# HyeonwooNoh/RAU_VQA

Hardware: AMD Instinct MI355X
Metric: QA-pairs/sec fwd+bwd, Ours_SS 8-step RAU, batch 256, 14x14x512 (higher is better)
Workload: dtype f32; 1 GPU; Ours_SS 8-step RAU fwd+bwd, 14x14x512, configs[1]; batch_per_gpu=256, global_batch=256, T=26, feature_map=14x14x512, hops=8, parallelism=dp1, collective=none, hop_weights=SS (x nHop), arithmetic=f32 operands, f32 MFMA accumulate, dropout=train mode, Philox masks per step and rank, launch=eager, 3 streams

## Files before the change

### rau_vqa_amd/csrc/gemm_lin.hip

```cpp
#include <algorithm>
#include <cstdio>
#include <cstdlib>

#include "gemm_core.h"
#include "kernels.h"

namespace rau {

constexpr int BK = 32;
constexpr int BKS = 16;

static GemmParams lin_params(int M, int N, int K, const float* A, long lda, const float* W,
                             long ldw, float* C, long ldc, const LinOpts& o) {
  GemmParams P{};
  P.M = M; P.N = N; P.K = K;
  P.nk = (K + BK - 1) / BK;
  P.A = A; P.a_rs = lda;
  P.B = W; P.b_rs = ldw;
  P.C = C; P.c_rs = ldc;
  P.bias = o.bias; P.bias2 = o.bias2;
  P.addend = o.addend; P.add_rs = o.add_rs;
  P.accumulate = o.accumulate; P.act = o.act;
  P.ymul = o.ymul; P.y_rs = o.y_rs;
  P.emask = o.emask; P.emask_e0 = o.emask_e0; P.emscale = o.emscale;
  P.alpha = o.alpha;
  P.round16 = lin_bf16();
  return P;
}

static int skinny_splits(int M, int N, int K, const LinOpts& o) {
  if (!o.slab) return 1;
  const int tiles = ((M + 63) / 64) * ((N + 63) / 64);
  const int nk = (K + BKS - 1) / BKS;
  constexpr int target = 160;
  int s = (target + tiles - 1) / tiles;
  if (s > nk / 2) s = nk / 2;
  if (s < 1) s = 1;
  while (s > 1 && (size_t)s * M * N > o.slab_floats) --s;
  const int per = (nk + s - 1) / s;
  return (nk + per - 1) / per;
}

template <int ASRC, int BSRC>
static hipError_t lin_gemm(hipStream_t st, int M, int N, int K, const float* A, long lda,
                           const float* W, long ldw, float* C, long ldc, const LinOpts& o) {
  GemmParams P = lin_params(M, N, K, A, lda, W, ldw, C, ldc, o);
  if ((long)M * N >= 128L * 128 * 256 && !o.defer_splits)
    return launch_gemm<128, 128, BK, ASRC, BSRC, EPI_LIN>(st, P, 1);
  if (o.slab && skinny_dma_ok(M, K, lda, ldw, BSRC == SRC_RC, 1, &N, &A, &W)) {
    const int tiles = ((M + 63) / 64) * ((N + 63) / 64);
    const int s = skinny_dma_splits(M, K, tiles, (size_t)N, o.slab_floats);
    if ((size_t)s * M * N <= o.slab_floats && (s > 1 || o.defer_splits)) {
      const long off = 0;
      hipError_t e = skinny_dma(st, BSRC == SRC_RC, 1, M, K, &A, lda, &W, ldw, &N, o.slab, &off, s);
      if (e != hipSuccess) return e;
      if (o.defer_splits) {
        *o.defer_splits = s;
        return hipSuccess;
      }
      return lin_reduce_epilogue(st, M, N, s, o.slab, C, ldc, o);
    }
  }
#ifdef RAU_DEV_HOOKS
  if (std::getenv("RAU_LIN_TRACE"))
    std::fprintf(stderr, "lin_gemm fallback %s M=%d N=%d K=%d lda=%ld ldw=%ld slab=%d\n",
                 BSRC == SRC_RC ? "nn" : "nt", M, N, K, lda, ldw, o.slab != nullptr);
#endif
  P.nk = (K + BKS - 1) / BKS;
  const int s = skinny_splits(M, N, K, o);
  if (o.defer_splits) {
    if (!o.slab || (size_t)s * M * N > o.slab_floats) return hipErrorInvalidValue;
    P.C = o.slab;
    P.c_rs = N;
    P.slab_stride = (long)M * N;
    *o.defer_splits = s;
    return launch_gemm<64, 64, BKS, ASRC, BSRC, EPI_SLAB>(st, P, s);
  }
  if (s <= 1) return launch_gemm<64, 64, BKS, ASRC, BSRC, EPI_LIN>(st, P, 1);
  P.C = o.slab;
  P.c_rs = N;
  P.slab_stride = (long)M * N;
  hipError_t e = launch_gemm<64, 64, BKS, ASRC, BSRC, EPI_SLAB>(st, P, s);
  if (e != hipSuccess) return e;
  return lin_reduce_epilogue(st, M, N, s, o.slab, C, ldc, o);
}

hipError_t gemm_nt(hipStream_t st, int M, int N, int K, const float* A, long lda,
                   const float* W, long ldw, float* C, long ldc, const LinOpts& o) {
  return lin_gemm<SRC_KC, SRC_KC>(st, M, N, K, A, lda, W, ldw, C, ldc, o);
}

hipError_t gemm_nn(hipStream_t st, int M, int N, int K, const float* A, long lda,
                   const float* W, long ldw, float* C, long ldc, const LinOpts& o) {
  return lin_gemm<SRC_KC, SRC_RC>(st, M, N, K, A, lda, W, ldw, C, ldc, o);
}

template <int ASRC, int BSRC>
static hipError_t batched_deferred(hipStream_t st, int nb, int M, int N, int K,
                                   const float* const* A, long lda, const float* const* W,
                                   long ldw, float* slab, size_t slab_floats, int* splits) {
  if (nb < 1 || nb > 3) return hipErrorInvalidValue;
  {
    const int Ns[3] = {N, N, N};
    if (skinny_dma_ok(M, K, lda, ldw, BSRC == SRC_RC, nb, Ns, A, W)) {
      const int tiles = ((M + 63) / 64) * ((N + 63) / 64);
      const int s = skinny_dma_splits(M, K, nb * tiles, (size_t)nb * N, slab_floats);
      if ((size_t)nb * s * M * N <= slab_floats) {
        long off[3];
        for (int i = 0; i < nb; ++i) off[i] = (long)i * s * M * N;
        *splits = s;
        return skinny_dma(st, BSRC == SRC_RC, nb, M, K, A, lda, W, ldw, Ns, slab, off, s);
      }
    }
  }
#ifdef RAU_DEV_HOOKS
  if (std::getenv("RAU_LIN_TRACE"))
    std::fprintf(stderr, "batched fallback %s nb=%d M=%d N=%d K=%d slab_floats=%zu\n", BSRC == SRC_RC ? "nn" : "nt",
                 nb, M, N, K, slab_floats);
#endif
  LinOpts o;
  o.slab = slab;
  o.slab_floats = slab_floats / nb;
  GemmParams P = lin_params(M, N, K, A[0], lda, W[0], ldw, slab, N, o);
  P.nk = (K + BKS - 1) / BKS;
  const int s = skinny_splits(M, N, K, o);
  if ((size_t)nb * s * M * N > slab_floats) return hipErrorInvalidValue;
  P.nbatch = nb;
  for (int i = 0; i < nb; ++i) { P.Ab[i] = A[i]; P.Bb[i] = W[i]; }
  P.C = slab;
  P.c_rs = N;
  P.slab_stride = (long)M * N;
  P.slab_batch_stride = (long)s * M * N;
  *splits = s;
  return launch_gemm<64, 64, BKS, ASRC, BSRC, EPI_SLAB>(st, P, s);
}
hipError_t gemm_nt_batched_deferred(hipStream_t st, int nb, int M, int N, int K,
                                    const float* const* A, long lda, const float* const* W,
                                    long ldw, float* slab, size_t slab_floats, int* splits) {
  return batched_deferred<SRC_KC, SRC_KC>(st, nb, M, N, K, A, lda, W, ldw, slab, slab_floats, splits);
}
hipError_t gemm_nn_batched_deferred(hipStream_t st, int nb, int M, int N, int K,
                                    const float* const* A, long lda, const float* const* W,
                                    long ldw, float* slab, size_t slab_floats, int* splits) {
  return batched_deferred<SRC_KC, SRC_RC>(st, nb, M, N, K, A, lda, W, ldw, slab, slab_floats, splits);
}

hipError_t gemm_nt_hetero_deferred(hipStream_t st, int nb, int M, int K, const float* A, long lda,
                                   const float* const* W, long ldw, const int* N, float* slab,
                                   size_t slab_floats, int* splits, size_t* off) {
  if (nb < 1 || nb > 3) return hipErrorInvalidValue;
  int nmax = 0, tiles = 0;
  size_t nsum = 0;
  for (int i = 0; i < nb; ++i) {
    nmax = N[i] > nmax ? N[i] : nmax;
    tiles += ((M + 63) / 64) * ((N[i] + 63) / 64);
    nsum += (size_t)N[i];
  }
  {
    const float* As[3] = {A, A, A};
    if (skinny_dma_ok(M, K, lda, ldw, false, nb, N, As, W)) {
      const int s = skinny_dma_splits(M, K, tiles, nsum, slab_floats);
      if ((size_t)s * M * nsum <= slab_floats) {
        long o2[3];
        size_t acc = 0;
        for (int i = 0; i < nb; ++i) {
          o2[i] = (long)acc;
          off[i] = acc;
          acc += (size_t)s * M * N[i];
        }
        *splits = s;
        return skinny_dma(st, false, nb, M, K, As, lda, W, ldw, N, slab, o2, s);
      }
    }
  }
#ifdef RAU_DEV_HOOKS
  if (std::getenv("RAU_LIN_TRACE"))
    std::fprintf(stderr, "hetero fallback nb=%d M=%d K=%d N=%d,%d,%d\n", nb, M, K, N[0], nb > 1 ? N[1] : 0, nb > 2 ? N[2] : 0);
#endif
  const int nk = (K + BKS - 1) / BKS;
  int s = (160 * nb + tiles - 1) / tiles;
  if (s > nk / 2) s = nk / 2;
  if (s < 1) s = 1;
  while (s > 1 && (size_t)s * M * nsum > slab_floats) --s;
  if ((size_t)s * M * nsum > slab_floats) return hipErrorInvalidValue;
  {
    const int per = (nk + s - 1) / s;
    s = (nk + per - 1) / per;
  }
  LinOpts o;
  GemmParams P = lin_params(M, nmax, K, A, lda, W[0], ldw, slab, nmax, o);
  P.nk = nk;
  P.nbatch = nb;
  size_t acc = 0;
  for (int i = 0; i < nb; ++i) {
    P.Ab[i] = A;
    P.Bb[i] = W[i];
    P.Nb[i] = N[i];
    P.slab_off[i] = (long)acc;
    off[i] = acc;
    acc += (size_t)s * M * N[i];
  }
  *splits = s;
  return launch_gemm<64, 64, BKS, SRC_KC, SRC_KC, EPI_SLAB>(st, P, s);
}

static int tn_splits(int M, int N, int K) {
  const int tiles = ((M + 127) / 128) * ((N + 127) / 128);
  const int nk = (K + BK - 1) / BK;
  constexpr int target = 512;
  int s = target / tiles;
  if (s > nk / 8) s = nk / 8;
  if (s < 1) s = 1;
  const int per = (nk + s - 1) / s;
  return (nk + per - 1) / per;
}
size_t gemm_tn_slab_floats(int M, int N, int K) {
  const int s = tn_splits(M, N, K);
  return (s > 1 ? (size_t)s * M * N : 0) + (size_t)s * M;
}
hipError_t gemm_tn_acc(hipStream_t st, int M, int N, int K, const float* A, long lda,
                       const float* B, long ldb, float* C, long ldc, float* slab, float* dbias, int bf16) {
  LinOpts o;
  o.accumulate = 1;
  const int s = tn_splits(M, N, K);
  float* rs = dbias ? slab + (s > 1 ? (size_t)s * M * N : 0) : nullptr;
  hipError_t e;
  if (s <= 1) {
    GemmParams P = lin_params(M, N, K, A, lda, B, ldb, C, ldc, o);
    P.rs_out = rs;
    if (bf16)
      e = dbias ? launch_gemm<128, 128, BK, SRC_RC_SUM, SRC_RC, EPI_LIN, 1>(st, P, 1)
                : launch_gemm<128, 128, BK, SRC_RC, SRC_RC, EPI_LIN, 1>(st, P, 1);
    else
    e = dbias ? launch_gemm<128, 128, BK, SRC_RC_SUM, SRC_RC, EPI_LIN>(st, P, 1)
              : launch_gemm<128, 128, BK, SRC_RC, SRC_RC, EPI_LIN>(st, P, 1);
  } else {
    if (ldc != N) return hipErrorInvalidValue;
    GemmParams P = lin_params(M, N, K, A, lda, B, ldb, slab, N, o);
    P.slab_stride = (long)M * N;
    P.rs_out = rs;
    if (bf16)
      e = dbias ? launch_gemm<128, 128, BK, SRC_RC_SUM, SRC_RC, EPI_SLAB, 1>(st, P, s)
                : launch_gemm<128, 128, BK, SRC_RC, SRC_RC, EPI_SLAB, 1>(st, P, s);
    else
    e = dbias ? launch_gemm<128, 128, BK, SRC_RC_SUM, SRC_RC, EPI_SLAB>(st, P, s)
              : launch_gemm<128, 128, BK, SRC_RC, SRC_RC, EPI_SLAB>(st, P, s);
    if (e != hipSuccess) return e;
    e = splitk_reduce_acc(st, (size_t)M * N, s, slab, (size_t)M * N, C);
  }
  if (e != hipSuccess || !dbias) return e;
  return splitk_reduce_acc(st, (size_t)M, s, rs, (size_t)M, dbias);
}

static int group_splits(const TnProblem* pr, int np, int K) {
  int tiles = 0;
  for (int i = 0; i < np; ++i) tiles += ((pr[i].M + 127) / 128) * ((pr[i].N + 127) / 128);
  const int nk = (K + BK - 1) / BK;
  constexpr int target = 0;
  const int smax = std::max(1, nk / 16);
  int s = 1;
  if (target > 0) {
    s = (target + tiles / 2) / (tiles > 0 ? tiles : 1);
    s = std::min(std::max(s, 1), smax);
  } else {
    double best = -1.0;
    for (int c = 1; c <= smax; ++c) {
      const int wgs = tiles * c;
      const double eff = (double)wgs / (512.0 * ((wgs + 511) / 512));
      if (eff > best + 0.02) { best = eff; s = c; }
    }
  }
  const int per = (nk + s - 1) / s;
  return (nk + per - 1) / per;
}
size_t gemm_tn_group_slab_floats(const TnProblem* pr, int np, int K) {
  const int s = group_splits(pr, np, K);
  size_t n = 0;
  for (int i = 0; i < np; ++i) n += (size_t)s * ((size_t)pr[i].M * pr[i].N + pr[i].M);
  return n;
}

struct GroupReduce {
  int np, splits;
  long e0[kGroupMax + 1];
  long b0[kGroupMax + 1];
  const float* slab[kGroupMax]; const float* rs[kGroupMax];
  float* dst[kGroupMax]; float* db[kGroupMax];
  long mn[kGroupMax]; int m[kGroupMax];
};
__global__ void k_group_reduce_acc(const GroupReduce R) {
  const long nW = R.e0[R.np], nB = R.b0[R.np];
  for (long i = blockIdx.x * (long)blockDim.x + threadIdx.x; i < nW + nB;
       i += (long)gridDim.x * blockDim.x) {
    const bool bias = i >= nW;
    const long j = bias ? i - nW : i;
    const long* pre = bias ? R.b0 : R.e0;
    int p = 0;
    while (p + 1 < R.np && j >= pre[p + 1]) ++p;
    const long k = j - pre[p];
    if (bias) {
      if (!R.db[p]) continue;
      float v = R.db[p][k];
      for (int s = 0; s < R.splits; ++s) v += R.rs[p][(long)s * R.m[p] + k];
      R.db[p][k] = v;
    } else {
      float v = R.dst[p][k];
      for (int s = 0; s < R.splits; ++s) v += R.slab[p][(long)s * R.mn[p] + k];
      R.dst[p][k] = v;
    }
  }
}

hipError_t gemm_tn_group_acc(hipStream_t st, const TnProblem* pr, int np, int K, float* slab,
                             size_t slab_floats, int bf16) {
  if (np < 1 || np > kGroupMax) return hipErrorInvalidValue;
  if (gemm_tn_group_slab_floats(pr, np, K) > slab_floats) return hipErrorInvalidValue;
  const int s = group_splits(pr, np, K);
  GroupParams G{};
  GroupReduce R{};
  G.np = np; G.K = K;
  G.nk = (K + BK - 1) / BK;
  G.nk_per_split = (G.nk + s - 1) / s;
  R.np = np; R.splits = s;
  float* w = slab;
  int wg = 0;
  for (int i = 0; i < np; ++i) {
    GroupProb& q = G.p[i];
    q.A = pr[i].A; q.lda = pr[i].lda; q.B = pr[i].B; q.ldb = pr[i].ldb;
    q.M = pr[i].M; q.N = pr[i].N;
    q.tiles_m = (q.M + 127) / 128; q.tiles_n = (q.N + 127) / 128;
    q.slab = w;
    w += (size_t)s * q.M * q.N;
    q.rs_out = w;
    w += (size_t)s * q.M;
    G.wg0[i] = wg;
    wg += q.tiles_m * q.tiles_n * s;
    R.slab[i] = q.slab; R.rs[i] = q.rs_out; R.dst[i] = pr[i].C; R.db[i] = pr[i].dbias;
    R.mn[i] = (long)q.M * q.N; R.m[i] = q.M;
    R.e0[i + 1] = R.e0[i] + R.mn[i];
    R.b0[i + 1] = R.b0[i] + q.M;
  }
  G.wg0[np] = wg;
  if (bf16)
    hipLaunchKernelGGL((gemm_group_kernel<128, 128, BK, SRC_RC_SUM, SRC_RC, 1>), dim3(wg), dim3(256), 0,
                       st, G);
  else
  hipLaunchKernelGGL((gemm_group_kernel<128, 128, BK, SRC_RC_SUM, SRC_RC>), dim3(wg), dim3(256), 0,
                     st, G);
  hipError_t e = hipGetLastError();
  if (e != hipSuccess) return e;
  const long n = R.e0[np] + R.b0[np];
  const int blocks = (int)std::min<long>((n + 255) / 256, 2048);
  hipLaunchKernelGGL(k_group_reduce_acc, dim3(blocks), dim3(256), 0, st, R);
  return hipGetLastError();
}

}
```

### rau_vqa_amd/csrc/kernels.h

```cpp
#pragma once
#include <hip/hip_runtime.h>
#include <stddef.h>
#include <stdint.h>

#include "../../include/rau.h"

namespace rau {

constexpr long kMaxSplits = 4096;
constexpr hipError_t kSplitStateError = hipErrorIllegalState;
void split_ws_register(const float* base, size_t floats);
void split_ws_unregister(const float* base);
bool split_span_ok(const float* slab, long nsplit, size_t per_split_floats);

struct LinOpts {
  const float* bias = nullptr;
  const float* bias2 = nullptr;
  const float* addend = nullptr;
  long add_rs = 0;
  int accumulate = 0;
  int act = 0;
  const float* ymul = nullptr;
  long y_rs = 0;
  const uint32_t* emask = nullptr;
  size_t emask_e0 = 0;
  float emscale = 1.f;
  float alpha = 1.f;
  float* slab = nullptr;
  size_t slab_floats = 0;
  int* defer_splits = nullptr;
};
hipError_t gemm_nt(hipStream_t st, int M, int N, int K, const float* A, long lda,
                   const float* W, long ldw, float* C, long ldc, const LinOpts& o);
hipError_t gemm_nn(hipStream_t st, int M, int N, int K, const float* A, long lda,
                   const float* W, long ldw, float* C, long ldc, const LinOpts& o);
hipError_t gemm_nt_batched_deferred(hipStream_t st, int nb, int M, int N, int K,
                                    const float* const* A, long lda, const float* const* W,
                                    long ldw, float* slab, size_t slab_floats, int* splits);
hipError_t gemm_nn_batched_deferred(hipStream_t st, int nb, int M, int N, int K,
                                    const float* const* A, long lda, const float* const* W,
                                    long ldw, float* slab, size_t slab_floats, int* splits);
hipError_t gemm_nt_hetero_deferred(hipStream_t st, int nb, int M, int K, const float* A, long lda,
                                   const float* const* W, long ldw, const int* N, float* slab,
                                   size_t slab_floats, int* splits, size_t* off);
size_t gemm_tn_slab_floats(int M, int N, int K);
hipError_t gemm_tn_acc(hipStream_t st, int M, int N, int K, const float* A, long lda,
                       const float* B, long ldb, float* C, long ldc, float* slab,
                       float* dbias = nullptr, int bf16 = 0);

struct TnProblem {
  int M, N; const float* A; long lda; const float* B; long ldb; float* C; float* dbias;
};
size_t gemm_tn_group_slab_floats(const TnProblem* pr, int np, int K);
hipError_t gemm_tn_group_acc(hipStream_t st, const TnProblem* pr, int np, int K, float* slab,
                             size_t slab_floats, int bf16 = 0);

hipError_t conv_embed_fwd(hipStream_t st, int nB, int D, int S, int M, const float* X,
                          const float* WiT , const float* bi, float* I, int bf16 = 0,
                          int one_per_cu = 0 );
hipError_t conv_embed_fwd_b16(hipStream_t st, int nB, int D, int S, int M, const void* X16,
                              const void* WiT16, const float* bi, float* I);
hipError_t conv_att_pre_b16(hipStream_t st, int nB, int M, int S, int A, const float* I,
                            const void* WpT16, const float* bp, float* Pout);
hipError_t conv_att_pre(hipStream_t st, int nB, int M, int S, int A, const float* I,
                        const float* WpT , const float* bp, float* P, int bf16 = 0,
                        int one_per_cu = 0);
bool conv_sample_ok(int S, int which);
hipError_t conv_sample(hipStream_t st, int epi, int nB, int M, int K, int S, const float* Wt,
                       long w_rs, const float* X, long x_bs, float* C, long c_bs,
                       const float* bias, int act, const float* dj, const float* av,
                       const float* Y = nullptr, float* rs = nullptr, int c16 = 0);
bool conv_wide_ok(int M, int K, int S, long w_rs);
hipError_t conv_wide(hipStream_t st, int epi, int nB, int M, int K, int S, const float* Wt, long w_rs,
                     const float* X, long x_bs, float* C, long c_bs, const float* bias, int act,
                     const float* dj, const float* av, const float* Y, float* rs, int c16, int per_cu);
hipError_t transpose2d(hipStream_t st, int rows, int cols, const float* in, float* out,
                       void* out16 = nullptr);
hipError_t conv_att_dgrad(hipStream_t st, int nB, int M, int S, int A, const float* dS,
                          const float* Wp, const float* dj, const float* a, float* dI,
                          int bf16 = 0);
bool conv_dz_fused_ok(int S, int M, int bf16);
hipError_t conv_att_dgrad_dz(hipStream_t st, int nB, int M, int S, int A, const float* dS,
                             const float* Wp, const float* dj, const float* a, const float* I,
                             float* dZ, float* rs, int dz16 = 0,
                             int bf16 = 0,
                             int ds16 = 0,
                             int light = 0);
bool dgrad16_ok(int M, int K, int S, long w_rs);
hipError_t dgrad16(hipStream_t st, int nB, int M, int K, int S, const float* Wt, long w_rs,
                   const void* X, long x_bs, void* C, long c_bs, const float* dj, const float* av,
                   const float* Y, float* rs, int c16, int x16 = 0 );
bool dgrad_dma_ok(int M, int K, int S, long w_rs);
hipError_t dgrad_dma(hipStream_t st, int nB, int M, int K, int S, const float* Wt, long w_rs,
                     const float* X, long x_bs, float* C, long c_bs, const float* dj, const float* av,
                     const float* Y, float* rs);
hipError_t conv_att_wgrad_ds16(hipStream_t st, int nB, int M, int S, int A, const void* dS16,
                               const float* I, float* dWp, float* slab);
hipError_t conv_embed_dgrad(hipStream_t st, int nB, int D, int S, int M, const float* dZ,
                            const float* Wi, float* dX);
size_t conv_wgrad_slab_floats(int nB, int rowsA, int rowsB, int S);
bool wgrad16_ok(int ra, int rb, int S);
size_t wgrad16_slab_floats(int nB, int ra, int rb, int S);
hipError_t wgrad16(hipStream_t st, int nB, int ra, int rb, int S, const void* A16, long a_bs,
                   const void* B16, long b_bs, float* dW, float* slab);
bool skinny_dma_ok(int M, int K, long lda, long ldb, bool brc, int nprob, const int* N,
                   const float* const* A, const float* const* B);
int skinny_dma_splits(int M, int K, int tiles_all, size_t cols_all, size_t slab_floats);
void skinny_dma_set_deep(int on);
void lin_set_bf16(int on);
int lin_bf16();
hipError_t skinny_dma(hipStream_t st, bool brc, int nprob, int M, int K, const float* const* A,
                      long lda, const float* const* B, long ldb, const int* N, float* slab,
                      const long* off, int splits);
bool wgrad_dma_ok(int ra, int rb, int S);
hipError_t wgrad_dma(hipStream_t st, int nB, int ra, int rb, int S, const float* A, long a_bs,
                     const float* B, long b_bs, float* dW, float* slab, int splits);
hipError_t conv_att_wgrad(hipStream_t st, int nB, int M, int S, int A, const float* dS,
                          const float* I, float* dWp, float* slab, int bf16 = 0);
hipError_t conv_embed_wgrad(hipStream_t st, int nB, int D, int S, int M, const float* dI,
                            const float* I, const float* X, float* dWi, float* slab,
                            int bf16 = 0, float* dbi = nullptr ,
                            int dz_final = 0 );
hipError_t conv_embed_wgrad_b16(hipStream_t st, int nB, int D, int S, int M, const void* dZ16,
                                const void* X16, float* dWi, float* slab);

enum GateOrder { GATES_ATT = 0 ,
                 GATES_DEEP = 1  };

hipError_t fill_masks(hipStream_t st, uint64_t seed, uint32_t site, uint32_t step, float p,
                      size_t n, uint32_t* bits, const uint64_t* key_dev = nullptr);
hipError_t embed_fwd(hipStream_t st, int rows, int E, int V, const float* emb, const int32_t* tokens,
                     const uint32_t* mask, float mscale, float* we, size_t mask_e0 = 0);
hipError_t embed_bwd_rows(hipStream_t st, int rows, int E, int V, const int32_t* tokens, const float* dwe,
                          const float* we, const uint32_t* mask, size_t mask_e0, float mscale,
                          float* gE);
hipError_t lstm_fwd(hipStream_t st, int order, int nB, int R, float* g4, const float* c_prev,
                    long cp_rs, float* c, long c_rs, float* h, long h_rs, float* tanhc,
                    float* drop_out, const uint32_t* mask, size_t mask_e0, float mscale,
                    const float* slab = nullptr, int nsplit = 0);
hipError_t lstm_bwd(hipStream_t st, int order, int nB, int R, const float* gates,
                    const float* c_prev, long cp_rs, const float* tanhc, const float* dh,
                    long dh_rs, const float* dh2, const float* dc_next, float* dsum,
                    float* dc_prev, const int32_t* lens, int t, const float* dq_c,
                    const float* dq_h, long dq_rs, const float* slab = nullptr, int nsplit = 0);
struct LstmFwdCell {
  float* g4;
  int has_input;
  const float* b1; const float* b2;
  const float* slab; int nsplit;
  const float* c_prev; long cp_rs;
  float* c; long c_rs; float* h; long h_rs; float* tanhc;
  float* drop_out; const uint32_t* mask; size_t mask_e0; float mscale;
};
struct LstmFwdCells { int n; LstmFwdCell c[2]; };
hipError_t lstm_fwd_multi(hipStream_t st, int order, int nB, int R, const LstmFwdCells& cells);
struct EncWsParams {
  int B, R, TL, P;
  float *G1, *G2, *h1, *c1, *tc1, *x2, *h2, *c2, *tc2;
  const float *Wh1, *Wi2, *Wh2, *bi2, *bh2;
  const uint32_t* mask; float mscale;
  unsigned* cnt; int* err;
  int bf16 = 0;
};
bool enc_ws_ok(int B, int R);
int enc_ws_workgroups(int B);
bool enc_ws_coresident(int B, int blocks_per_cu, int n_cus);
bool enc_ws_fits_device(int B);
hipError_t enc_ws_forward(hipStream_t st, int order, EncWsParams Q);
struct LstmBwdCell {
  const float* gates; const float* c_prev; long cp_rs; const float* tanhc;
  const float* slabA; int nA;
  const float* slabB; int nBp;
  const uint32_t* maskB; size_t maskB_e0; float mscaleB;
  const float* dc_next; float* dsum; float* dc_prev;
  int t; const float* dq_c; const float* dq_h;
};
struct LstmBwdCells { int n; const int32_t* lens; long dq_rs; LstmBwdCell c[2]; };
hipError_t lstm_bwd_multi(hipStream_t st, int order, int nB, int R, const LstmBwdCells& cells);
struct AttPartials { int u_ns = 0; const float* u_bias = nullptr; int z_ns = 0; const float* z_bias = nullptr; int SL = 0; float* u_out = nullptr; int waves = 0;
                     const int32_t* img = nullptr; };
hipError_t att_fwd_fused(hipStream_t st, int nB, int M, int A, int S, const float* P,
                         const float* u, const float* ws, const float* bs, const float* zm,
                         const float* I, const float* qf, float* T, float* a, float* jv,
                         const AttPartials& ap = AttPartials());
hipError_t att_bwd_fused(hipStream_t st, int nB, int M, int A, int S, const float* I,
                         const float* dj, const float* a, const float* da_lin,
                         const float* ws, float* T_to_dS, float* dz, float* du, float* dwsp,
                         const float* Psrc = nullptr ,
                         const float* u = nullptr,
                         int da_ns = 0, int SL = 0, const float* da_add = nullptr,
                         void* dS16 = nullptr,
                         int waves_hint = 0 );
bool att_bwd_dma_ok(int M, int A, int S, int waves_hint = 0);
size_t att_split_part_floats(int nB, int S);
hipError_t att_fwd_split(hipStream_t st, int nB, int M, int A, int S, const float* P,
                         const float* u, const float* ws, const float* bs, const float* zm,
                         const float* I, const float* qf, float* a, float* jv, float* part,
                         const AttPartials& ap = AttPartials());
hipError_t att_bwd_split(hipStream_t st, int nB, int M, int A, int S, const float* I,
                         const float* dj, const float* a, const float* da_lin, const float* ws,
                         float* T_to_dS, float* dz, float* du, float* dwsp, const float* Psrc,
                         const float* u, float* part, int da_ns = 0, int SL = 0,
                         const float* da_add = nullptr);
inline bool feat_type_ok(int ft) { return ft == RAU_FEAT_F32 || ft == RAU_FEAT_F16 || ft == RAU_FEAT_BF16; }
hipError_t dropout_features(hipStream_t st, int H, size_t per_hop, const void* X,
                            const uint32_t* mask, float mscale, float* xd, size_t mask_e0 = 0,
                            int SL = 0, int Sp = 0, int ft = RAU_FEAT_F32);
hipError_t dropout_features_gen(hipStream_t st, uint64_t seed, uint32_t site, uint32_t step, float p,
// ... 58 lines not shown
```

### rau_vqa_amd/csrc/rau_ctx.hip

```cpp
#include "rau_ctx.h"

static thread_local char g_err[512] = "";
int fail(int code, const char* fmt, ...) {
  va_list ap;
  va_start(ap, fmt);
  vsnprintf(g_err, sizeof(g_err), fmt, ap);
  va_end(ap);
  return code;
}

static int prof_collect(rau_ctx* ctx) {
  if (ctx->precs.empty()) return 0;
  HIPC(hipStreamSynchronize(ctx->st));
  HIPC(hipStreamSynchronize(ctx->st2));
  HIPC(hipStreamSynchronize(ctx->st3));
  if (ctx->stc) HIPC(hipStreamSynchronize(ctx->stc));
  FILE* tl = nullptr;
  if (const char* p = std::getenv("RAU_PROF_TIMELINE")) tl = std::fopen(p, "a");
  for (auto& r : ctx->precs) {
    float ms = 0.f;
    hipEventElapsedTime(&ms, r.a, r.b);
    if (tl) {
      float t0 = 0.f;
      hipEventElapsedTime(&t0, ctx->precs[0].a, r.a);
// ... 1825 lines not shown
  const uint32_t* m_mf = mk(RAU_MASK_MF);
  if (HA > 0 && !ctx->dpre_fwd) {
    LINOPTS(o);
    o.emask = m_mf;
    o.emask_e0 = 0;
    o.emscale = sc(RAU_MASK_MF);
    RUN("head_dgrad", gflop(HA * B, M, K), 0,
        gemm_nn(st, HA * B, M, K, ctx->dl, K, ctx->cls.W, M, ctx->dpre, M, o));
    LINOPTS(o2);
    RUN("head_dgrad", gflop(HA * B, R, M), 0,
        gemm_nn(st, HA * B, R, M, ctx->dpre, M, ctx->lstm_out.W, R, ctx->dhn, R, o2));
  }
  const float* dc_next = nullptr;
  float* dh_part = nullptr;
  int dh_part_ns = 0;
  ctx->ds16_step = ctx->dS16 && !ctx->I_shared && !ctx->att_split_env && conv_dz_fused_ok(S, M, ctx->bf16);
  struct Ds16Reset { rau_ctx* c; ~Ds16Reset() { c->ds16_step = false; } } ds16_reset{ctx};
  bool dq_side = false;
  int dq_rows_left = HA;
  for (int h = HA - 1; h >= 0; --h) {
    float* dc_out = ctx->dcn[h & 1];
    {
      HopGrad g{};
      g.dl = ctx->dl + (size_t)h * B * K;
      g.dc_next = dc_next;
      g.dh_next = nullptr;
      g.dc_out = dc_out;
      g.dh_out = nullptr;
      g.dpre_ready = 1;
      g.dhn_all = ctx->dhn;
      g.dh_part = dh_part;
      g.dh_part_ns = dh_part_ns;
      g.dh_part_out = &dh_part;
      g.dh_part_ns_out = &dh_part_ns;
      g.ev_conv_ready = (gsz[h] && (seam_mask() & 2)) ? ctx->evK[h] : nullptr;
      g.dh_prev_dead = h == 0;
      if (int rc = hop_backward(ctx, h, ctx->cc + (size_t)h * BR_,
                                ctx->I + (ctx->I_shared ? 0 : (size_t)h * BM_ * S), g))
        return rc;
    }
    dc_next = dc_out;
    if (gsz[h] && h > 0 && side_split(ctx)) {
      const int nh = std::min(h + gsz[h], HA) - h;
      HIPC(hipEventRecord(ctx->evK[h], st));
      HIPC(hipStreamWaitEvent(ctx->st3, ctx->evK[h], 0));
      LinOpts o;
      o.slab = ctx->slab3; o.slab_floats = ctx->slab3_floats;
      RUNS(ctx->st3, "q_proj_dgrad", gflop(nh * B, Q, M), 0,
           gemm_nn(ctx->st3, nh * B, Q, M, ctx->dqt + (size_t)h * BM_, M, ctx->q_proj.W, Q,
                   ctx->dQD + (size_t)h * B * Q, Q, o));
      HIPC(hipEventRecord(ctx->evDq, ctx->st3));
      dq_side = true;
      dq_rows_left = h;
    }
    if (gsz[h]) {
      hipStream_t sb = ctx->st2;
      if (!(seam_mask() & 2)) HIPC(hipEventRecord(ctx->evK[h], st));
      HIPC(hipStreamWaitEvent(sb, ctx->evK[h], 0));
      if (!ctx->I_shared) {
        const int nH = (std::min(h + gsz[h], HA) - h) * B;
        const size_t hb = (size_t)h * B;
        const int dzf = conv_dz_fused_ok(S, M, ctx->bf16);
        if (dzf)
          RUNS(sb, "conv_att_dgrad", gflop(M, (double)nH * S, A),
               ((double)nH * A * S + 3.0 * nH * M * S) * 4,
               conv_att_dgrad_dz(sb, nH, M, S, A,
                                 ctx->ds16_step ? (const float*)((const uint16_t*)ctx->dS16 + hb * A * S)
                                                : ctx->T + hb * A * S,
                                 ctx->att_i.W, ctx->dj + hb * M,
                                 ctx->a + hb * S, ctx->I + hb * M * S,
                                 ctx->xd16 ? (float*)((uint16_t*)ctx->dZ + hb * M * S) : ctx->dZ + hb * M * S,
                                 ctx->dbi_part + hb * M, ctx->xd16 ? 1 : 0, ctx->bf16, ctx->ds16_step ? 1 : 0,
                                 chain_bound(ctx) ? 1 : 0));
        else
          RUNS(sb, "conv_att_dgrad", gflop(M, (double)nH * S, A),
               ((double)nH * A * S + 2.0 * nH * M * S) * 4,
               conv_att_dgrad(sb, nH, M, S, A, ctx->T + hb * A * S, ctx->att_i.W, ctx->dj + hb * M,
                              ctx->a + hb * S, ctx->dZ + hb * M * S, ctx->bf16));
        {
          if (ctx->ds16_step)
            RUNS(sb, "conv_att_wgrad", gflop(A, M, (double)nH * S),
                 (double)nH * A * S * 2 + (double)nH * M * S * 4,
                 conv_att_wgrad_ds16(sb, nH, M, S, A, (const uint16_t*)ctx->dS16 + hb * A * S,
                                     ctx->I + hb * M * S, ctx->att_i.dW, ctx->slab2));
          else
          RUNS(sb, "conv_att_wgrad", gflop(A, M, (double)nH * S),
               ((double)nH * A * S + (double)nH * M * S) * 4,
               conv_att_wgrad(sb, nH, M, S, A, ctx->T + hb * A * S, ctx->I + hb * M * S,
                              ctx->att_i.dW, ctx->slab2, ctx->bf16));
        }
        if (ctx->xd16 && dzf)
          RUNS(sb, "conv_embed_wgrad", gflop(M, D, (double)nH * S),
               (double)nH * M * S * 2 + (double)nH * D * S * 2,
               conv_embed_wgrad_b16(sb, nH, D, S, M, (const uint16_t*)ctx->dZ + hb * M * S,
                                    (const uint16_t*)ctx->xd16 + hb * D * S, ctx->i_embed.dW, ctx->slab2));
        else
          RUNS(sb, "conv_embed_wgrad", gflop(M, D, (double)nH * S),
               ((double)nH * M * S * (dzf ? 1 : 2) + (double)nH * D * S) * 4,
               conv_embed_wgrad(sb, nH, D, S, M, ctx->dZ + hb * M * S, ctx->I + hb * M * S,
                                  ctx->xd + hb * D * S, ctx->i_embed.dW, ctx->slab2, ctx->bf16,
                                  ctx->i_embed.db, dzf));
        if (dzf && h == 0)
          RUNS(sb, "colsum", 0, (double)HA * B * M * 4,
               colsum_acc(sb, HA * B, M, ctx->dbi_part, M, ctx->i_embed.db, ctx->coltmp2));
      } else {
        for (int hh2 = 0; hh2 < HA; ++hh2) {
          float* Th2 = ctx->T + (size_t)hh2 * B * A * S;
          float* dZh = ctx->dZ + (size_t)hh2 * BM_ * S;
          RUNS(sb, "conv_att_dgrad", gflop(M, (double)B * S, A), ((double)B * A * S + 2.0 * BM_ * S) * 4,
               conv_att_dgrad(sb, B, M, S, A, Th2, ctx->att_i.W, ctx->dj + (size_t)hh2 * BM_,
                              ctx->a + (size_t)hh2 * BS_, dZh, ctx->bf16));
          RUNS(sb, "conv_att_wgrad", gflop(A, M, (double)B * S), ((double)B * A * S + BM_ * S) * 4,
               conv_att_wgrad(sb, B, M, S, A, Th2, ctx->I, ctx->att_i.dW, ctx->slab2, ctx->bf16));
          RUNS(sb, "conv_embed_wgrad", gflop(M, D, (double)B * S), (BM_ * S + (double)B * D * S) * 4,
               conv_embed_wgrad(sb, B, D, S, M, dZh, ctx->I, ctx->xw, ctx->i_embed.dW, ctx->slab2,
                                ctx->bf16, ctx->i_embed.db));
        }
      }
    }
  }
  {
    LINOPTS(o);
    if (dq_rows_left > 0)
      RUN("q_proj_dgrad", gflop(dq_rows_left * B, Q, M), 0,
          gemm_nn(st, dq_rows_left * B, Q, M, ctx->dqt, M, ctx->q_proj.W, Q, ctx->dQD, Q, o));
    if (dq_side) HIPC(hipStreamWaitEvent(st, ctx->evDq, 0));
    RUN("dq_reduce", 0, (double)HA * B * Q * 4,
        dq_reduce(st, HA, (size_t)B * Q, ctx->dQD, m_q, sc(RAU_MASK_Q), ctx->dq));
  }
  {
    hipStream_t sb = ctx->st2;
    HIPC(hipEventRecord(ctx->evD, sb));
  }
  HIPC(hipEventRecord(ctx->evW, st));
  static const int wg_env = [] { const char* e = std::getenv("RAU_WG_BULK"); return e ? std::atoi(e) : -1; }();
  const int wg_bulk = side_split(ctx) ? 0 : wg_env >= 0 ? wg_env : (chain_bound(ctx) ? 0 : 1);
  auto mult_wgrads = [&]() -> int {
    hipStream_t sw = (wg_bulk & 1) ? ctx->st2 : ctx->st3;
    HIPC(hipStreamWaitEvent(sw, ctx->evW, 0));
    const int rows = HA * B;
    if (rows == 0) {
      HIPC(hipEventRecord(ctx->evM3, sw));
      return 0;
    }
    {
      TnProblem pr[13];
      const int np = mult_wgrad_problems(ctx, pr);
      double fl = 0;
      for (int i = 0; i < np; ++i) fl += gflop(pr[i].M, pr[i].N, rows);
      float* ws = (wg_bulk & 1) ? ctx->slab2 : ctx->slab3;
      const size_t ws_floats = (wg_bulk & 1) ? ctx->slab2_floats : ctx->slab3_floats;
      RUNS(sw, "wgrad_gemm", fl, 0, gemm_tn_group_acc(sw, pr, np, rows, ws, ws_floats, ctx->bf16 == 1));
    }
    float* ct = (wg_bulk & 1) ? ctx->coltmp2 : ctx->coltmp3;
    RUNS(sw, "colsum", 0, (double)rows * A * 4, colsum_acc(sw, rows, A, ctx->dwsp, A, ctx->att_score.dW, ct));
    HIPC(hipMemsetAsync(ctx->tmpS, 0, S * sizeof(float), sw));
    RUNS(sw, "colsum", 0, (double)rows * S * 4, colsum_acc(sw, rows, SL, ctx->dz, S, ctx->tmpS, ct));
    RUNS(sw, "colsum", 0, S * 4.0, colsum_acc(sw, SL, 1, ctx->tmpS, 1, ctx->att_score.db, ct));
    RUNS(sw, "colsum", 0, (double)rows * A * 4, colsum_acc(sw, rows, A, ctx->du, A, ctx->att_i.db, ct));
    HIPC(hipEventRecord(ctx->evM3, sw));
    return 0;
  };
  if (int rc = mult_wgrads()) return rc;

  if (TL > 0) {
    const int rows = TL * B;
    const size_t G4 = (size_t)B * 4 * Rq;
    auto enc_wgrads = [&](int t_lo, int t_hi, hipEvent_t ev) -> int {
      if (t_hi <= t_lo) return 0;
      hipStream_t sw = (wg_bulk & 2) ? ctx->st2 : ctx->st3;
      HIPC(hipEventRecord(ev, st));
      HIPC(hipStreamWaitEvent(sw, ev, 0));
      const size_t r0 = (size_t)t_lo * B;
      const int nr = (t_hi - t_lo) * B;
      TnProblem pr[13];
      const int np = enc_wgrad_problems(ctx, r0, pr);
      double fl = 0;
      for (int i = 0; i < np; ++i) fl += gflop(pr[i].M, pr[i].N, nr);
      float* ws = (wg_bulk & 2) ? ctx->slab2 : ctx->slab3;
      const size_t ws_floats = (wg_bulk & 2) ? ctx->slab2_floats : ctx->slab3_floats;
      RUNS(sw, "wgrad_gemm", fl, 0, gemm_tn_group_acc(sw, pr, np, nr, ws, ws_floats, ctx->bf16 == 1));
      return 0;
    };
    const int hi = TL;
    for (int u = TL; u >= 0; --u) {
      const float* Ap[3];
      const float* Wp[3];
      int nb = 0, iq2 = -1, iqx = -1, iq1 = -1;
      if (u >= 1 && u + 1 <= TL) { Ap[nb] = ctx->dG2 + (size_t)u * G4; Wp[nb] = ctx->h2h[1].W; iq2 = nb++; }
      if (u + 1 <= TL) { Ap[nb] = ctx->dG2 + (size_t)u * G4; Wp[nb] = ctx->i2h[1].W; iqx = nb++; }
      if (u + 2 <= TL) { Ap[nb] = ctx->dG1 + (size_t)(u + 1) * G4; Wp[nb] = ctx->h2h[0].W; iq1 = nb++; }
      int nsp = 0;
      if (nb > 0)
        RUN("enc_h2h_dgrad", gflop(B, Rq, 4 * Rq) * nb, 0,
            gemm_nn_batched_deferred(st, nb, B, Rq, 4 * Rq, Ap, 4 * Rq, Wp, Rq, ctx->slab,
                                     ctx->slab_floats, &nsp));
      LstmBwdCells cells{};
      cells.lens = ctx->lens_d;
      cells.dq_rs = Q;
      if (u >= 1) {
        LstmBwdCell& C2 = cells.c[cells.n++];
        C2.gates = ctx->G2 + (size_t)(u - 1) * G4;
        C2.c_prev = ctx->c2 + (size_t)(u - 1) * BRq; C2.cp_rs = Rq;
        C2.tanhc = ctx->tc2 + (size_t)(u - 1) * BRq;
        C2.slabA = iq2 >= 0 ? ctx->slab + (size_t)iq2 * nsp * BRq : nullptr;
        C2.nA = iq2 >= 0 ? nsp : 0;
        C2.slabB = nullptr; C2.nBp = 0; C2.maskB = nullptr; C2.maskB_e0 = 0; C2.mscaleB = 1.f;
        C2.dc_next = u < TL ? ctx->edc[1][(u + 1) & 1] : nullptr;
        C2.dsum = ctx->dG2 + (size_t)(u - 1) * G4;
        C2.dc_prev = ctx->edc[1][u & 1];
        C2.t = u; C2.dq_c = ctx->dq + 2 * Rq; C2.dq_h = ctx->dq + 3 * Rq;
      }
      if (u + 1 <= TL) {
        const int t = u + 1;
        LstmBwdCell& C1 = cells.c[cells.n++];
        C1.gates = ctx->G1 + (size_t)u * G4;
        C1.c_prev = ctx->c1 + (size_t)u * BRq; C1.cp_rs = Rq;
        C1.tanhc = ctx->tc1 + (size_t)u * BRq;
        C1.slabA = iq1 >= 0 ? ctx->slab + (size_t)iq1 * nsp * BRq : nullptr;
        C1.nA = iq1 >= 0 ? nsp : 0;
        C1.slabB = ctx->slab + (size_t)iqx * nsp * BRq;
        C1.nBp = nsp;
        C1.maskB = m_rnn; C1.maskB_e0 = (size_t)u * BRq; C1.mscaleB = sc(RAU_MASK_RNN);
        C1.dc_next = t < TL ? ctx->edc[0][(t + 1) & 1] : nullptr;
        C1.dsum = ctx->dG1 + (size_t)u * G4;
        C1.dc_prev = ctx->edc[0][t & 1];
        C1.t = t; C1.dq_c = ctx->dq; C1.dq_h = ctx->dq + Rq;
      }
      RUN("lstm_bwd", 0, BRq * 4.0 * 12 * cells.n, lstm_bwd_multi(st, GATES_DEEP, B, Rq, cells));
    }
    {
      LINOPTS(o);
      RUN("enc_i2h_dgrad", gflop(rows, E, 4 * Rq), 0,
          gemm_nn(st, rows, E, 4 * Rq, ctx->dG1, 4 * Rq, ctx->i2h[0].W, E, ctx->dwe, E, o));
    }
    RUN("embed_bwd", 0, (double)rows * E * 12,
        embed_bwd(st, ctx->capturing ? c.T * B : ctx->nuniq, E, ctx->utok, ctx->ustart, ctx->upos, ctx->dwe, ctx->we, m_we,
                  sc(RAU_MASK_WE), ctx->grp[RAU_GROUP_EMBED].g));
    if (int rc = enc_wgrads(0, hi, ctx->evE)) return rc;
  }
  HIPC(hipEventRecord(ctx->evW3, ctx->st3));
  HIPC(hipStreamWaitEvent(st, ctx->evW3, 0));
  if (wg_bulk) HIPC(hipEventRecord(ctx->evD, ctx->st2));
  HIPC(hipStreamWaitEvent(st, ctx->evD, 0));
  HIPC(hipEventRecord(ctx->evEnd, st));
  ctx->bwd_done = true;
  ctx->graph_last = false;
  return RAU_OK;
}

int rau_graph_step(rau_ctx* ctx, const float* hop_w, int zero_grads_first) {
  NEED(ctx && hop_w, "null argument");
  if (!ctx->have_batch || !ctx->have_labels)
    return fail(RAU_ERR_STATE, "rau_graph_step: needs a batch with labels (rau_set_batch)");
  if (ctx->prof_on) return fail(RAU_ERR_STATE, "rau_graph_step: profiling must be off");
  const int H = ctx->cfg.H;
  int HA = 0;
  for (int h = 0; h < H; ++h)
    if (hop_w[h] != 0.f) HA = h + 1;
  uint64_t key = (uint64_t)ctx->mode | ((uint64_t)ctx->max_len << 2) | ((uint64_t)HA << 12) |
                 ((uint64_t)(zero_grads_first != 0) << 22);
  for (int i = 0; i < 5; ++i) key |= (uint64_t)ctx->mexplicit[i] << (24 + i);
  key |= (uint64_t)ctx->cur_slot << 30;
  key |= (uint64_t)ctx->feat_type << 32;
  key |= (uint64_t)(ctx->n_images > 0) << 34;
  key |= (uint64_t)ctx->slot[ctx->cur_slot].bank << 35;
  if (int rc = upload_hop_weights(ctx, hop_w)) return rc;
  ctx->mg_valid = false;
  hipGraphExec_t exec = nullptr;
  for (auto& g : ctx->graphs)
    if (g.first == key) exec = g.second;
  if (!exec) {
    hipGraph_t graph = nullptr;
    HIPC(hipStreamBeginCapture(ctx->st, hipStreamCaptureModeRelaxed));
    ctx->capturing = true;
    int rc = zero_grads_first ? rau_zero_grads(ctx) : 0;
    if (!rc) rc = rau_forward(ctx);
    if (!rc) rc = rau_backward(ctx, hop_w);
    ctx->capturing = false;
    hipError_t e = hipStreamEndCapture(ctx->st, &graph);
    if (rc) {
      if (graph) hipGraphDestroy(graph);
      return rc;
    }
    if (e != hipSuccess)
      return fail(RAU_ERR_DEVICE, "hipStreamEndCapture: %s", hipGetErrorString(e));
    e = hipGraphInstantiate(&exec, graph, nullptr, nullptr, 0);
    hipGraphDestroy(graph);
    if (e != hipSuccess)
      return fail(RAU_ERR_DEVICE, "hipGraphInstantiate: %s", hipGetErrorString(e));
    ctx->graphs.push_back({key, exec});
  }
  HIPC(hipGraphLaunch(exec, ctx->st));
  if (ctx->n_images) {
    ctx->x_valid = true;
    ctx->x_slot = ctx->cur_slot;
    ctx->x_serial = ctx->slot_serial[ctx->cur_slot];
  }
  HIPC(hipEventRecord(ctx->evEnd, ctx->st));
  merge_record(ctx);
  ctx->fwd_done = false;
  ctx->bwd_done = true;
  ctx->graph_last = true;
  return RAU_OK;
}

int rau_wait_grads(rau_ctx* ctx, int group, void* hip_stream) {
  if (int rc = check_group(ctx, group)) return rc;
  if (!ctx->bwd_done) return fail(RAU_ERR_STATE, "rau_wait_grads: no rau_backward to wait for");
  hipStream_t s = (hipStream_t)hip_stream;
  if (group == RAU_GROUP_MULT && !ctx->graph_last) {
    HIPC(hipStreamWaitEvent(s, ctx->evD, 0));
    HIPC(hipStreamWaitEvent(s, ctx->evM3, 0));
// ... 242 lines not shown
```

Before: 27630 QA-pairs/s.

## Add dedicated LDS-pipelined wgrad GEMM kernel and move colsums to separate stream

Adds a new split-K weight-gradient kernel for f32 TN grouped problems. It uses direct global-to-LDS loads, a three-stage LDS ring, hand-scheduled ds_read_b128 and MFMA 16x16x4 issue, and fused row-sum accumulation. Eligible problems (M, N divisible by 4, non-bf16) are routed to it instead of the generic group GEMM, with slab offsets padded to 4 floats for aligned float4 stores. The mult-wgrad colsum reductions now always run on stream st3, so they can overlap the GEMM on the other stream, joined back through an event. This adds an alignment requirement on the slab and a more complex cross-stream dependency.

```diff
diff --git a/rau_vqa_amd/csrc/gemm_lin.hip b/rau_vqa_amd/csrc/gemm_lin.hip
--- a/rau_vqa_amd/csrc/gemm_lin.hip
+++ b/rau_vqa_amd/csrc/gemm_lin.hip
@@ -1,4 +1,5 @@
 #include <algorithm>
+#include <cstdint>
 #include <cstdio>
 #include <cstdlib>
 
@@ -273,10 +274,11 @@
   const int per = (nk + s - 1) / s;
   return (nk + per - 1) / per;
 }
+static size_t up4(size_t n) { return (n + 3) & ~(size_t)3; }
 size_t gemm_tn_group_slab_floats(const TnProblem* pr, int np, int K) {
   const int s = group_splits(pr, np, K);
   size_t n = 0;
-  for (int i = 0; i < np; ++i) n += (size_t)s * ((size_t)pr[i].M * pr[i].N + pr[i].M);
+  for (int i = 0; i < np; ++i) n += up4((size_t)s * pr[i].M * pr[i].N) + up4((size_t)s * pr[i].M);
   return n;
 }
 
@@ -316,37 +318,46 @@
   if (np < 1 || np > kGroupMax) return hipErrorInvalidValue;
   if (gemm_tn_group_slab_floats(pr, np, K) > slab_floats) return hipErrorInvalidValue;
   const int s = group_splits(pr, np, K);
-  GroupParams G{};
+  GroupParams G{}, D{};
   GroupReduce R{};
-  G.np = np; G.K = K;
-  G.nk = (K + BK - 1) / BK;
-  G.nk_per_split = (G.nk + s - 1) / s;
+  for (GroupParams* g : {&G, &D}) {
+    g->K = K;
+    g->nk = (K + BK - 1) / BK;
+    g->nk_per_split = (g->nk + s - 1) / s;
+  }
   R.np = np; R.splits = s;
   float* w = slab;
-  int wg = 0;
   for (int i = 0; i < np; ++i) {
-    GroupProb& q = G.p[i];
+    GroupParams& g = (!bf16 && wgrad_lin_ok(pr[i].M, pr[i].N)) ? D : G;
+    GroupProb& q = g.p[g.np];
     q.A = pr[i].A; q.lda = pr[i].lda; q.B = pr[i].B; q.ldb = pr[i].ldb;
     q.M = pr[i].M; q.N = pr[i].N;
     q.tiles_m = (q.M + 127) / 128; q.tiles_n = (q.N + 127) / 128;
     q.slab = w;
-    w += (size_t)s * q.M * q.N;
+    w += up4((size_t)s * q.M * q.N);
     q.rs_out = w;
-    w += (size_t)s * q.M;
-    G.wg0[i] = wg;
-    wg += q.tiles_m * q.tiles_n * s;
+    w += up4((size_t)s * q.M);
+    g.wg0[g.np + 1] = g.wg0[g.np] + q.tiles_m * q.tiles_n * s;
+    ++g.np;
     R.slab[i] = q.slab; R.rs[i] = q.rs_out; R.dst[i] = pr[i].C; R.db[i] = pr[i].dbias;
     R.mn[i] = (long)q.M * q.N; R.m[i] = q.M;
     R.e0[i + 1] = R.e0[i] + R.mn[i];
     R.b0[i + 1] = R.b0[i] + q.M;
   }
-  G.wg0[np] = wg;
-  if (bf16)
-    hipLaunchKernelGGL((gemm_group_kernel<128, 128, BK, SRC_RC_SUM, SRC_RC, 1>), dim3(wg), dim3(256), 0,
-                       st, G);
-  else
-  hipLaunchKernelGGL((gemm_group_kernel<128, 128, BK, SRC_RC_SUM, SRC_RC>), dim3(wg), dim3(256), 0,
-                     st, G);
+  if (D.np > 0) {
+    if ((reinterpret_cast<uintptr_t>(slab) & 15) != 0) return hipErrorInvalidValue;
+    hipError_t e = wgrad_lin_group(st, D);
+    if (e != hipSuccess) return e;
+  }
+  if (G.np > 0) {
+    const int wg = G.wg0[G.np];
+    if (bf16)
+      hipLaunchKernelGGL((gemm_group_kernel<128, 128, BK, SRC_RC_SUM, SRC_RC, 1>), dim3(wg), dim3(256), 0,
+                         st, G);
+    else
+      hipLaunchKernelGGL((gemm_group_kernel<128, 128, BK, SRC_RC_SUM, SRC_RC>), dim3(wg), dim3(256), 0,
+                         st, G);
+  }
   hipError_t e = hipGetLastError();
   if (e != hipSuccess) return e;
   const long n = R.e0[np] + R.b0[np];
diff --git a/rau_vqa_amd/csrc/kernels.h b/rau_vqa_amd/csrc/kernels.h
--- a/rau_vqa_amd/csrc/kernels.h
+++ b/rau_vqa_amd/csrc/kernels.h
@@ -54,6 +54,10 @@
 size_t gemm_tn_group_slab_floats(const TnProblem* pr, int np, int K);
 hipError_t gemm_tn_group_acc(hipStream_t st, const TnProblem* pr, int np, int K, float* slab,
                              size_t slab_floats, int bf16 = 0);
+struct GroupParams;
+bool wgrad_lin_ok(int M, int N);
+hipError_t wgrad_lin_group(hipStream_t st, const GroupParams& G);
+int wgrad_lin_bank_conflicts(void);
 
 hipError_t conv_embed_fwd(hipStream_t st, int nB, int D, int S, int M, const float* X,
                           const float* WiT , const float* bi, float* I, int bf16 = 0,
diff --git a/rau_vqa_amd/csrc/rau_ctx.hip b/rau_vqa_amd/csrc/rau_ctx.hip
--- a/rau_vqa_amd/csrc/rau_ctx.hip
+++ b/rau_vqa_amd/csrc/rau_ctx.hip
@@ -2001,13 +2001,19 @@
       const size_t ws_floats = (wg_bulk & 1) ? ctx->slab2_floats : ctx->slab3_floats;
       RUNS(sw, "wgrad_gemm", fl, 0, gemm_tn_group_acc(sw, pr, np, rows, ws, ws_floats, ctx->bf16 == 1));
     }
-    float* ct = (wg_bulk & 1) ? ctx->coltmp2 : ctx->coltmp3;
-    RUNS(sw, "colsum", 0, (double)rows * A * 4, colsum_acc(sw, rows, A, ctx->dwsp, A, ctx->att_score.dW, ct));
-    HIPC(hipMemsetAsync(ctx->tmpS, 0, S * sizeof(float), sw));
-    RUNS(sw, "colsum", 0, (double)rows * S * 4, colsum_acc(sw, rows, SL, ctx->dz, S, ctx->tmpS, ct));
-    RUNS(sw, "colsum", 0, S * 4.0, colsum_acc(sw, SL, 1, ctx->tmpS, 1, ctx->att_score.db, ct));
-    RUNS(sw, "colsum", 0, (double)rows * A * 4, colsum_acc(sw, rows, A, ctx->du, A, ctx->att_i.db, ct));
-    HIPC(hipEventRecord(ctx->evM3, sw));
+    hipStream_t sc_ = ctx->st3;
+    float* ct = ctx->coltmp3;
+    if (sc_ != sw) HIPC(hipStreamWaitEvent(sc_, ctx->evW, 0));
+    RUNS(sc_, "colsum", 0, (double)rows * A * 4, colsum_acc(sc_, rows, A, ctx->dwsp, A, ctx->att_score.dW, ct));
+    HIPC(hipMemsetAsync(ctx->tmpS, 0, S * sizeof(float), sc_));
+    RUNS(sc_, "colsum", 0, (double)rows * S * 4, colsum_acc(sc_, rows, SL, ctx->dz, S, ctx->tmpS, ct));
+    RUNS(sc_, "colsum", 0, S * 4.0, colsum_acc(sc_, SL, 1, ctx->tmpS, 1, ctx->att_score.db, ct));
+    RUNS(sc_, "colsum", 0, (double)rows * A * 4, colsum_acc(sc_, rows, A, ctx->du, A, ctx->att_i.db, ct));
+    HIPC(hipEventRecord(ctx->evM3, sc_));
+    if (sw != sc_) {
+      HIPC(hipStreamWaitEvent(sw, ctx->evM3, 0));
+      HIPC(hipEventRecord(ctx->evM3, sw));
+    }
     return 0;
   };
   if (int rc = mult_wgrads()) return rc;
diff --git a/rau_vqa_amd/csrc/wgrad_lin.hip b/rau_vqa_amd/csrc/wgrad_lin.hip
--- /dev/null
+++ b/rau_vqa_amd/csrc/wgrad_lin.hip
@@ -0,0 +1,231 @@
+#include <type_traits>
+#include <utility>
+
+#include "common.h"
+#include "gemm_core.h"
+#include "kernels.h"
+
+namespace rau {
+
+namespace {
+
+constexpr int LT = 128;
+constexpr int LKS = 16;
+constexpr int LPART = LKS * LT;
+constexpr int LSTAGE = 2 * LPART;
+constexpr int LNST = 3;
+constexpr int LSMEM = 14336;
+
+typedef __attribute__((address_space(3))) void* lds_ptr_t;
+typedef const __attribute__((address_space(1))) void* glb_ptr_t;
+
+__device__ __attribute__((aligned(16))) float g_zero16[4] = {0.f, 0.f, 0.f, 0.f};
+
+template <int OFF>
+__device__ __forceinline__ void lds_read128(f32x4& dst, uint32_t addr) {
+  asm volatile("ds_read_b128 %0, %1 offset:%2" : "=v"(dst) : "v"(addr), "n"(OFF) : "memory");
+}
+
+__global__ __launch_bounds__(256, 2) void k_wgrad_lin(const GroupParams G) {
+  __shared__ __attribute__((aligned(16))) float smem[LSMEM];
+  const int tid = threadIdx.x, l = tid & 63;
+  const int w = __builtin_amdgcn_readfirstlane(tid >> 6);
+  const int wm = w & 1, wn = w >> 1;
+
+  const int v = xcd_remap((int)blockIdx.x, (int)gridDim.x);
+  int pi = 0;
+#pragma unroll 1
+  while (pi + 1 < G.np && v >= G.wg0[pi + 1]) ++pi;
+  const GroupProb& q = G.p[pi];
+  const int local = v - G.wg0[pi];
+  const int tiles = q.tiles_m * q.tiles_n;
+  const int split = local / tiles, tile = local - split * tiles;
+  int tm, tn;
+  if (q.tiles_n <= q.tiles_m) { tm = tile / q.tiles_n; tn = tile - tm * q.tiles_n; }
+  else { tn = tile / q.tiles_m; tm = tile - tn * q.tiles_m; }
+  const int M = q.M, N = q.N;
+  const int m0 = tm * LT, n0 = tn * LT;
+  const int k_lo = split * G.nk_per_split * 32;
+  int k_hi = k_lo + G.nk_per_split * 32;
+  if (k_hi > G.K) k_hi = G.K;
+  const int nst = k_hi > k_lo ? (k_hi - k_lo + LKS - 1) / LKS : 0;
+
+  const int lrow = l >> 5, lcol = 4 * (l & 31);
+  const bool cokA = m0 + lcol < M, cokB = n0 + lcol < N;
+  uint32_t voff[4];
+  int vrow[4];
+#pragma unroll
+  for (int n = 0; n < 4; ++n) {
+    const int i = w + 4 * n;
+    vrow[n] = 2 * (i & 7) + lrow;
+    voff[n] = (uint32_t)(((long)vrow[n] * (n < 2 ? q.lda : q.ldb) + lcol) * 4);
+  }
+  const char* const zero = reinterpret_cast<const char*>(g_zero16);
+  const char* ap = reinterpret_cast<const char*>(q.A + (size_t)k_lo * q.lda + m0);
+  const char* bp = reinterpret_cast<const char*>(q.B + (size_t)k_lo * q.ldb + n0);
+  const size_t astep = (size_t)LKS * q.lda * 4, bstep = (size_t)LKS * q.ldb * 4;
+  const char *ia = ap, *ib = bp;
+  int ik = k_lo, islot = 0;
+  auto issue_slot = [&](int n) {
+    const bool a = n < 2;
+    const bool ok = (a ? cokA : cokB) && ik + vrow[n] < k_hi;
+    const char* src = ok ? (a ? ia : ib) + voff[n] : zero;
+    const int i = w + 4 * n;
+    __builtin_amdgcn_global_load_lds((glb_ptr_t)src,
+                                     (lds_ptr_t)(smem + islot * LSTAGE + (a ? 0 : LPART) + 256 * (i & 7)),
+                                     16, 0, 0);
+  };
+  auto next_stage = [&]() {
+    ia += astep; ib += bstep; ik += LKS;
+    islot = islot == LNST - 1 ? 0 : islot + 1;
+  };
+
+  f32x4 acc[4][4];
+#pragma unroll
+  for (int i = 0; i < 4; ++i)
+#pragma unroll
+    for (int j = 0; j < 4; ++j) acc[i][j] = f32x4{0.f, 0.f, 0.f, 0.f};
+  typedef float f32x2 __attribute__((ext_vector_type(2)));
+  f32x2 asum_lo = f32x2{0.f, 0.f}, asum_hi = f32x2{0.f, 0.f};
+  const bool do_sum = wn == 0 && tn == 0;
+
+  const int x = l & 15, g = l >> 4;
+  const uint32_t lds0 = (uint32_t)(size_t)(lds_ptr_t)smem;
+  const uint32_t fa = lds0 + (uint32_t)(g * LT + wm * 64 + 4 * x) * 4;
+  const uint32_t fb = lds0 + (uint32_t)(LPART + g * LT + wn * 64 + 4 * x) * 4;
+  constexpr int KG = 4 * LT * 4;
+
+  if (nst > 0) {
+#pragma unroll
+    for (int n = 0; n < 4; ++n) issue_slot(n);
+    next_stage();
+  }
+  if (nst > 1) {
+#pragma unroll
+    for (int n = 0; n < 4; ++n) issue_slot(n);
+    next_stage();
+  }
+  int rslot = 0;
+#pragma unroll 1
+  for (int s = 0; s < nst; ++s) {
+    if (s + 1 < nst)
+      asm volatile("s_waitcnt vmcnt(4)" ::: "memory");
+    else
+      asm volatile("s_waitcnt vmcnt(0)" ::: "memory");
+    __builtin_amdgcn_s_barrier();
+    const bool more = s + 2 < nst;
+    const uint32_t so = (uint32_t)(rslot * LSTAGE) * 4;
+    rslot = rslot == LNST - 1 ? 0 : rslot + 1;
+    f32x4 a4[2], b4[2];
+    auto mma = [&](int set) {
+      asm volatile("v_pk_add_f32 %0, %0, %2\n\tv_pk_add_f32 %1, %1, %3"
+                   : "+v"(asum_lo), "+v"(asum_hi)
+                   : "v"(__builtin_shufflevector(a4[set], a4[set], 0, 1)),
+                     "v"(__builtin_shufflevector(a4[set], a4[set], 2, 3)));
+#pragma unroll
+      for (int i = 0; i < 4; ++i)
+#pragma unroll
+        for (int j = 0; j < 4; ++j)
+          acc[i][j] = __builtin_amdgcn_mfma_f32_16x16x4f32(a4[set][i], b4[set][j], acc[i][j], 0, 0, 0);
+    };
+    lds_read128<0>(a4[0], fa + so);
+    lds_read128<0>(b4[0], fb + so);
+    lds_read128<KG>(a4[1], fa + so);
+    lds_read128<KG>(b4[1], fb + so);
+    asm volatile("s_waitcnt lgkmcnt(2)" ::: "memory");
+    __builtin_amdgcn_sched_barrier(0);
+    mma(0);
+    if (more) issue_slot(0);
+    __builtin_amdgcn_sched_barrier(0);
+    lds_read128<2 * KG>(a4[0], fa + so);
+    lds_read128<2 * KG>(b4[0], fb + so);
+    asm volatile("s_waitcnt lgkmcnt(2)" ::: "memory");
+    __builtin_amdgcn_sched_barrier(0);
+    mma(1);
+    if (more) issue_slot(1);
+    __builtin_amdgcn_sched_barrier(0);
+    lds_read128<3 * KG>(a4[1], fa + so);
+    lds_read128<3 * KG>(b4[1], fb + so);
+    asm volatile("s_waitcnt lgkmcnt(2)" ::: "memory");
+    __builtin_amdgcn_sched_barrier(0);
+    mma(0);
+    if (more) issue_slot(2);
+    __builtin_amdgcn_sched_barrier(0);
+    asm volatile("s_waitcnt lgkmcnt(0)" ::: "memory");
+    __builtin_amdgcn_sched_barrier(0);
+    mma(1);
+    if (more) { issue_slot(3); next_stage(); }
+    __builtin_amdgcn_sched_barrier(0);
+  }
+
+  if (do_sum) {
+    float asum[4] = {asum_lo[0], asum_lo[1], asum_hi[0], asum_hi[1]};
+#pragma unroll
+    for (int c = 0; c < 4; ++c) {
+      float t = asum[c];
+      t += __shfl_xor(t, 16, 64);
+      t += __shfl_xor(t, 32, 64);
+      asum[c] = t;
+    }
+    const int m = m0 + wm * 64 + 4 * x;
+    if (g == 0 && m < M)
+      *reinterpret_cast<float4*>(q.rs_out + (size_t)split * M + m) = make_float4(asum[0], asum[1], asum[2], asum[3]);
+  }
+  float* C = q.slab + (size_t)split * M * N;
+  const int cb = n0 + wn * 64 + 4 * x;
+  if (cb < N) {
+#pragma unroll
+    for (int i = 0; i < 4; ++i)
+#pragma unroll
+      for (int r = 0; r < 4; ++r) {
+        const int ca = m0 + wm * 64 + 4 * (4 * g + r) + i;
+        if (ca < M)
+          *reinterpret_cast<float4*>(C + (size_t)ca * N + cb) =
+              make_float4(acc[i][0][r], acc[i][1][r], acc[i][2][r], acc[i][3][r]);
+        __builtin_amdgcn_sched_barrier(0);
+      }
+  }
+}
+
+}
+
+bool wgrad_lin_ok(int M, int N) {
+  static const bool off = std::getenv("RAU_WGRAD_LIN_OFF") != nullptr;
+  return !off && M > 0 && N > 0 && M % 4 == 0 && N % 4 == 0;
+}
+
+hipError_t wgrad_lin_group(hipStream_t st, const GroupParams& G) {
+  const int wg = G.wg0[G.np];
+  if (wg <= 0) return hipSuccess;
+  hipLaunchKernelGGL(k_wgrad_lin, dim3(wg), dim3(256), 0, st, G);
+  return hipGetLastError();
+}
+
+int wgrad_lin_bank_conflicts(void) {
+  static const int groups[4][16] = {{0, 1, 2, 3, 12, 13, 14, 15, 20, 21, 22, 23, 24, 25, 26, 27},
+                                    {4, 5, 6, 7, 8, 9, 10, 11, 16, 17, 18, 19, 28, 29, 30, 31},
+                                    {32, 33, 34, 35, 44, 45, 46, 47, 52, 53, 54, 55, 56, 57, 58, 59},
+                                    {36, 37, 38, 39, 40, 41, 42, 43, 48, 49, 50, 51, 60, 61, 62, 63}};
+  int worst = 0;
+  for (int part = 0; part < 2; ++part)
+    for (int wh = 0; wh < 2; ++wh)
+      for (int kk = 0; kk < LKS / 4; ++kk)
+        for (int slot = 0; slot < LNST; ++slot)
+          for (const auto& grp : groups) {
+            int seen[64][16], cnt[64] = {};
+            for (int li : grp) {
+              const int x = li & 15, g = li >> 4;
+              const int word = slot * LSTAGE + part * LPART + (4 * kk + g) * LT + wh * 64 + 4 * x;
+              for (int c = 0; c < 4; ++c) {
+                const int bank = (word + c) % 64;
+                bool dup = false;
+                for (int t = 0; t < cnt[bank]; ++t) dup = dup || seen[bank][t] == word + c;
+                if (!dup) seen[bank][cnt[bank]++] = word + c;
+              }
+            }
+            for (int b = 0; b < 64; ++b) worst = cnt[b] - 1 > worst ? cnt[b] - 1 : worst;
+          }
+  return worst;
+}
+
+}
```

New measurement: 27630 QA-pairs/s, median of 2. No clear change (+0.0%).
